# ZhonghuaYi/FocusFlow_official

Measured on AMD Instinct MI355X. Metric: frame-pairs/sec FF-RAFT 384x512 iters=12, higher is better.
Workload: dtype f32 via fp16x3 split operands on the f16 MFMA pipe (f32 accumulate, fp32-level accuracy); 1 GPU; FF-RAFT forward (test_mode), 8 pairs/GPU 384x512, iters=12, fp32 correlation pyramid, random-init weights, ORB-like masks (BASELINE configs[1]); pairs_per_gpu=8, corr_pyramid=fp32, conv_precision=f16x3, hipgraph=False, skip_unused_upsample=False, parallelism=dp1 (independent shards, no collective)

## Files before the change

### focusflow_official_amd/csrc/conv_patch.hip

```cpp
#include <algorithm>
#include <cstdlib>
#include "ff_common.h"

namespace {

typedef float f32x16 __attribute__((ext_vector_type(16)));
typedef float f32x4 __attribute__((ext_vector_type(4)));
typedef _Float16 f16x8 __attribute__((ext_vector_type(8)));
typedef _Float16 f16x4 __attribute__((ext_vector_type(4)));

constexpr int TW = 16, ROWB = 128;
constexpr int ROWP = 144;
__device__ __forceinline__ int PI16(int i) { return (i >= 4 && i < 12) ? 2 * (i - 4) : (i < 4 ? 2 * i + 1 : 2 * (i - 12) + 9); }
__device__ __forceinline__ int KG16(int g) { return ((g & 1) << 1) | (g >> 1); }


struct PArgs {
    FFConvParams p;
    int Cin, nci;
    int tiles_x, tiles_y, n_tiles;
    long long w_row_bytes;
    int nci_split;
};

__device__ __forceinline__ void split4(const f32x4 v, f16x4& h0, f16x4& h1) {
#pragma unroll
    for (int j = 0; j < 4; ++j) {
        const _Float16 a = (_Float16)v[j];
        h0[j] = a;
        h1[j] = (_Float16)(v[j] - (float)a);
    }
}

template <int TERMS, int NITEM, int TM, int TN, int ABL, int WB, bool PIN = false, bool INORM = false, bool SPLITK = false, bool MF16 = false, int EPI = 0, bool STATS = false>
__device__ __forceinline__ void conv_patch_body(const PArgs& a) {
    constexpr int TH = 4 * TM, BN = 64 * TN, NW = 2 * TN;
    extern __shared__ __attribute__((aligned(16))) char smem[];
    const FFConvParams& p = a.p;
    float xs, xinv;
    ff::input_scale(p.x_amax, xs, xinv);
    xs *= ff::XSPLIT; xinv *= ff::SPLIT_INV;
    const int KH = p.KH, KW = p.KW, PH = TH + KH - 1, PW = TW + KW - 1, NPIX = PH * PW;
    char* sP = smem;
    char* sW = smem + ((NPIX * ROWP + 255) & ~255);

    const int tid = threadIdx.x, lane = tid & 63, wave = tid >> 6;
    const int wm = wave >> 1, wn = wave & 1;
    const int H = p.H, W = p.W;
    int bid = blockIdx.x;
    const int nt = bid % a.n_tiles; bid /= a.n_tiles;
    const int tx = bid % a.tiles_x; bid /= a.tiles_x;
    const int ty = bid % a.tiles_y;
    const int bimg = bid / a.tiles_y;
    const int y0 = ty * TH, x0 = tx * TW, n0 = nt * BN;

    const long long pix_total = (long long)p.B * H * W;
    __amdgpu_buffer_rsrc_t rs0 = __builtin_amdgcn_make_buffer_rsrc(const_cast<float*>(p.x[0]), 0, (int)(pix_total * p.x_ld[0] * 4), 0x00020000);
    __amdgpu_buffer_rsrc_t rs1 = __builtin_amdgcn_make_buffer_rsrc(const_cast<float*>(p.x[1] ? p.x[1] : p.x[0]), 0, p.x[1] ? (int)(pix_total * p.x_ld[1] * 4) : 0, 0x00020000);
    __amdgpu_buffer_rsrc_t rs2 = __builtin_amdgcn_make_buffer_rsrc(const_cast<float*>(p.x[2] ? p.x[2] : p.x[0]), 0, p.x[2] ? (int)(pix_total * p.x_ld[2] * 4) : 0, 0x00020000);
    __amdgpu_buffer_rsrc_t rsw = __builtin_amdgcn_make_buffer_rsrc(const_cast<float*>(p.w), 0, (int)((long long)p.Cout * a.w_row_bytes), 0x00020000);
    const int c0 = p.x_c[0], c01 = p.x_c[0] + p.x_c[1];

    int ppix[NITEM];
    int prow[NITEM];
#pragma unroll
    for (int i = 0; i < NITEM; ++i) {
        const int item = tid + 256 * i;
        const int px = item >> 3;
        ppix[i] = -1;
        prow[i] = px;
        if (px < NPIX) {
            const int yy = y0 - p.pad_h + px / PW, xx = x0 - p.pad_w + px % PW;
            if ((unsigned)yy < (unsigned)H && (unsigned)xx < (unsigned)W) ppix[i] = (bimg * H + yy) * W + xx;
        }
    }
    const int kq = tid & 7;
    int woff[NW];
#pragma unroll
    for (int i = 0; i < NW; ++i) {
        const int n = n0 + (tid >> 3) + 32 * i;
        woff[i] = n < p.Cout ? (int)(n * a.w_row_bytes) + kq * 16 : 0x7fffffff;
    }

    f32x4 rp[NITEM], rw[NW];
    f32x4 nmul = {1.f, 1.f, 1.f, 1.f}, nadd = {0.f, 0.f, 0.f, 0.f};
    auto load_patch = [&](int c) {
        int ci0 = c * 32;
        if (INORM) {
            const long long t = (long long)bimg * a.Cin + ci0 + kq * 4;
            nmul = *reinterpret_cast<const f32x4*>(p.in_scale + t);
            nadd = *reinterpret_cast<const f32x4*>(p.in_shift + t);
        }
        __amdgpu_buffer_rsrc_t rs;
        int ldb;
        if (ci0 < c0) { rs = rs0; ldb = p.x_ld[0] * 4; }
        else if (ci0 < c01) { rs = rs1; ldb = p.x_ld[1] * 4; ci0 -= c0; }
        else { rs = rs2; ldb = p.x_ld[2] * 4; ci0 -= c01; }
        const int cib = (ci0 + kq * 4) * 4;
#pragma unroll
        for (int i = 0; i < NITEM; ++i) {
            const int off = ppix[i] >= 0 ? ppix[i] * ldb + cib : 0x7fffffff;
            rp[i] = __builtin_bit_cast(f32x4, __builtin_amdgcn_raw_buffer_load_b128(rs, off, 0, 0));
        }
    };
    auto store_patch = [&]() {
        const int pc = MF16 ? KG16(kq >> 1) : kq >> 1, half = (kq & 1) * 8;
#pragma unroll
        for (int i = 0; i < NITEM; ++i) {
            const int row = prow[i];
            if (row < NPIX) {
                f16x4 h0, h1;
                f32x4 v = rp[i];
                if (INORM) {
                    v = __builtin_elementwise_fma(v, nmul, nadd);
                    if (p.in_act == FF_ACT_RELU) {
#pragma unroll
                        for (int j = 0; j < 4; ++j) v[j] = v[j] < 0.f ? 0.f : v[j];
                    }
                    if (ppix[i] < 0) v = (f32x4){0.f, 0.f, 0.f, 0.f};
                }
                split4(v * xs, h0, h1);
                *reinterpret_cast<f16x4*>(sP + row * ROWP + pc * 16 + half) = h0;
                if (TERMS == 3) *reinterpret_cast<f16x4*>(sP + row * ROWP + 64 + pc * 16 + half) = h1;
            }
        }
    };
    auto load_w = [&](int kc) {
#pragma unroll
        for (int i = 0; i < NW; ++i)
            rw[i] = __builtin_bit_cast(f32x4, __builtin_amdgcn_raw_buffer_load_b128(rsw, woff[i], kc * ROWB, 0));
    };
    auto store_w = [&](int buf) {
        char* d = sW + buf * BN * ROWP;
#pragma unroll
        for (int i = 0; i < NW; ++i) {
            const int row = (tid >> 3) + 32 * i;
            if (MF16) *reinterpret_cast<f32x4*>(d + ((row & ~15) + PI16(row & 15)) * ROWP + ((kq & 4) | KG16(kq & 3)) * 16) = rw[i];
            else *reinterpret_cast<f32x4*>(d + row * ROWP + kq * 16) = rw[i];
        }
    };

    if constexpr (MF16) {
        constexpr int NU = 2 * TM, NV = 2 * TN;
        f32x4 acc[NV][NU];
#pragma unroll
        for (int v = 0; v < NV; ++v)
#pragma unroll
            for (int u = 0; u < NU; ++u) acc[v][u] = (f32x4){0.f, 0.f, 0.f, 0.f};
        const int i16 = lane & 15, g16 = lane >> 4, pcol = PI16(i16);
        const int ntaps = KH * KW;
        const char* xbase = sP + ((wm * NU) * PW + pcol) * ROWP + KG16(g16) * 16;
        const int wrow0 = (wn * TN * 32 + PI16(i16)) * ROWP + KG16(g16) * 16;
        const int c_beg = SPLITK ? (int)blockIdx.y * a.nci_split : 0;
        const int c_end = SPLITK ? min(c_beg + a.nci_split, a.nci) : a.nci;
        load_patch(c_beg);
        load_w(c_beg);
        int wbuf = 0;
        for (int c = c_beg; c < c_end; ++c) {
            __syncthreads();
            store_patch();
            store_w(wbuf);
            __syncthreads();
            if (c + 1 < c_end) load_patch(c + 1);
            for (int tap = 0; tap < ntaps; ++tap) {
                const bool last = tap + 1 == ntaps;
                const int next_kc = last ? (c + 1) : (tap + 1) * a.nci + c;
                if (!(last && c + 1 == c_end)) load_w(last ? c + 1 : next_kc);
                if (PIN) __builtin_amdgcn_sched_barrier(0);
                const int dy = tap / KW, dx = tap - dy * KW;
                const char* pa = xbase + (dy * PW + dx) * ROWP;
                const char* cW = sW + wbuf * BN * ROWP + wrow0;
                f16x8 w0[NV], w1[NV];
#pragma unroll
                for (int v = 0; v < NV; ++v) {
                    w0[v] = *reinterpret_cast<const f16x8*>(cW + v * 16 * ROWP);
                    if (TERMS == 3) w1[v] = *reinterpret_cast<const f16x8*>(cW + v * 16 * ROWP + 64);
                }
#pragma unroll
                for (int u = 0; u < NU; ++u) {
                    const f16x8 xa = *reinterpret_cast<const f16x8*>(pa + u * PW * ROWP);
                    f16x8 xb;
                    if (TERMS == 3) xb = *reinterpret_cast<const f16x8*>(pa + u * PW * ROWP + 64);
#pragma unroll
                    for (int v = 0; v < NV; ++v) {
                        acc[v][u] = __builtin_amdgcn_mfma_f32_16x16x32_f16(w0[v], xa, acc[v][u], 0, 0, 0);
                        if (TERMS == 3) {
                            acc[v][u] = __builtin_amdgcn_mfma_f32_16x16x32_f16(w1[v], xa, acc[v][u], 0, 0, 0);
                            acc[v][u] = __builtin_amdgcn_mfma_f32_16x16x32_f16(w0[v], xb, acc[v][u], 0, 0, 0);
                        }
                    }
                }
                if (!last) {
                    if (WB == 1) __syncthreads();
                    store_w(WB == 1 ? 0 : wbuf ^ 1);
                    __syncthreads();
                    if (WB == 2) wbuf ^= 1;
                }
            }
            if (WB == 2) wbuf ^= 1;
        }
        const int x = x0 + pcol;
        const bool vec_y = (p.y_ld & 3) == 0 && ff::aligned16(p.y);
        const bool vec_r = !p.res || ((p.res_ld & 3) == 0 && ff::aligned16(p.res));
#pragma unroll
        for (int v = 0; v < NV; ++v) {
            const int n4 = n0 + wn * TN * 32 + v * 16 + g16 * 4;
            if (n4 >= p.Cout) continue;
            const bool full = n4 + 3 < p.Cout;
            if constexpr (SPLITK) {
                float* ws = p.splitk_ws + (long long)blockIdx.y * pix_total * p.Cout;
#pragma unroll
                for (int u = 0; u < NU; ++u) {
                    const int y = y0 + wm * NU + u;
                    if (y >= H || x >= W) continue;
                    float* d = ws + (((long long)bimg * H + y) * W + x) * p.Cout + n4;
                    if (full && (p.Cout & 3) == 0) *reinterpret_cast<f32x4*>(d) = acc[v][u] * xinv;
                    else {
#pragma unroll
                        for (int r = 0; r < 4; ++r)
                            if (n4 + r < p.Cout) d[r] = acc[v][u][r] * xinv;
                    }
                }
                continue;
            }
            f32x4 bias = {0.f, 0.f, 0.f, 0.f}, cs = {1.f, 1.f, 1.f, 1.f}, ct = {0.f, 0.f, 0.f, 0.f};
#pragma unroll
            for (int r = 0; r < 4; ++r) {
                const int n = min(n4 + r, p.Cout - 1);
                if (p.bias) bias[r] = p.bias[n];
                if (p.ch_scale) { cs[r] = p.ch_scale[n]; ct[r] = p.ch_shift[n]; }
            }
            f32x4 vv[NU], rr[NU];
            long long po[NU];
#pragma unroll
            for (int u = 0; u < NU; ++u) {
                const int y = y0 + wm * NU + u;
                po[u] = (y < H && x < W) ? ((long long)bimg * H + y) * W + x : -1;
                f32x4 t = acc[v][u] * xinv + bias;
                t *= p.out_scale;
                if (p.ch_scale) t = t * cs + ct;
#pragma unroll
                for (int r = 0; r < 4; ++r) t[r] = ff::apply_act(t[r], p.act);
                vv[u] = t;
            }
            if (p.res) {
#pragma unroll
                for (int u = 0; u < NU; ++u) {
                    rr[u] = (f32x4){0.f, 0.f, 0.f, 0.f};
                    if (po[u] < 0) continue;
                    const float* rp2 = p.res + po[u] * p.res_ld + n4;
                    if (full && vec_r) rr[u] = *reinterpret_cast<const f32x4*>(rp2);
                    else {
#pragma unroll
                        for (int r = 0; r < 4; ++r)
                            if (n4 + r < p.Cout) rr[u][r] = rp2[r];
                    }
                }
#pragma unroll
                for (int u = 0; u < NU; ++u)
#pragma unroll
                    for (int r = 0; r < 4; ++r) vv[u][r] = ff::apply_act(vv[u][r] + rr[u][r], p.act_res);
            }
            if constexpr (EPI == FF_EP_GRU_RH) {
                if (n4 >= p.ep_split) {
#pragma unroll
                    for (int u = 0; u < NU; ++u) rr[u] = po[u] >= 0 ? *reinterpret_cast<const f32x4*>(p.ep_a + po[u] * p.ep_a_ld + (n4 - p.ep_split)) : (f32x4){0.f, 0.f, 0.f, 0.f};
#pragma unroll
                    for (int u = 0; u < NU; ++u)
#pragma unroll
                        for (int r = 0; r < 4; ++r) vv[u][r] = __fmul_rn(vv[u][r], rr[u][r]);
                }
            }
            if constexpr (EPI == FF_EP_GRU_BLEND) {
                f32x4 zz[NU];
#pragma unroll
                for (int u = 0; u < NU; ++u) {
                    zz[u] = po[u] >= 0 ? *reinterpret_cast<const f32x4*>(p.ep_a + po[u] * p.ep_a_ld + n4) : (f32x4){0.f, 0.f, 0.f, 0.f};
                    rr[u] = po[u] >= 0 ? *reinterpret_cast<const f32x4*>(p.ep_b + po[u] * p.ep_b_ld + n4) : (f32x4){0.f, 0.f, 0.f, 0.f};
                }
#pragma unroll
                for (int u = 0; u < NU; ++u)
#pragma unroll
                    for (int r = 0; r < 4; ++r)
                        vv[u][r] = __fadd_rn(__fmul_rn(__fsub_rn(1.f, zz[u][r]), rr[u][r]), __fmul_rn(zz[u][r], vv[u][r]));
            }
#pragma unroll
            for (int u = 0; u < NU; ++u) {
                if (po[u] < 0) continue;
                float* d = p.y + po[u] * p.y_ld + n4;
                if (full && vec_y) *reinterpret_cast<f32x4*>(d) = vv[u];
                else {
#pragma unroll
                    for (int r = 0; r < 4; ++r)
                        if (n4 + r < p.Cout) d[r] = vv[u][r];
                }
            }
        }
        return;
    }

    f32x16 acc[TM][TN];
#pragma unroll
    for (int i = 0; i < TM; ++i)
#pragma unroll
        for (int j = 0; j < TN; ++j)
#pragma unroll
            for (int r = 0; r < 16; ++r) acc[i][j][r] = 0.f;

    const int li = lane & 31, lh = lane >> 5;
    const int rot = (KW - 1) & 15;
    const int lrow = li >> 4, lcol = ((li & 15) - lrow * rot) & 15;
    const int ntaps = KH * KW;
    const int brow = wn * TN * 32 + li;
    const char* abase[TM];
#pragma unroll
    for (int t = 0; t < TM; ++t) abase[t] = sP + (((wm * TM + t) * 2 + lrow) * PW + lcol) * ROWP + lh * 16;

    f16x8 abl_f;
#pragma unroll
    for (int i = 0; i < 8; ++i) abl_f[i] = (_Float16)(0.37f + 0.01f * (float)((lane * 7 + i * 3) & 31));
    const int c_beg = SPLITK ? (int)blockIdx.y * a.nci_split : 0;
    const int c_end = SPLITK ? min(c_beg + a.nci_split, a.nci) : a.nci;
    load_patch(c_beg);
    load_w(c_beg);
    int wbuf = 0;
    for (int c = c_beg; c < c_end; ++c) {
        __syncthreads();
        if (ABL != 6 || c == c_beg) store_patch();
        store_w(wbuf);
        __syncthreads();
        if (c + 1 < c_end && ABL != 6) load_patch(c + 1);
        for (int tap = 0; tap < ntaps; ++tap) {
            const bool last = tap + 1 == ntaps;
            const int next_kc = last ? (c + 1) : (tap + 1) * a.nci + c;
            if (!(last && c + 1 == c_end) && ABL != 1 && ABL != 2) load_w(last ? c + 1 : next_kc);
            if (PIN) __builtin_amdgcn_sched_barrier(0);
            const int dy = tap / KW, dx = tap - dy * KW;
            const int tapoff = (dy * PW + dx) * ROWP;
            const char* cW = sW + wbuf * BN * ROWP + brow * ROWP + lh * 16;
#pragma unroll
            for (int s = 0; s < 2; ++s) {
                f16x8 a0[TM], a1[TM], b0[TN], b1[TN];
                if constexpr (ABL == 5) {
#pragma unroll
                    for (int t = 0; t < TM; ++t) { a0[t] = abl_f; a1[t] = abl_f; }
#pragma unroll
                    for (int j = 0; j < TN; ++j) { b0[j] = abl_f; b1[j] = abl_f; }
                    asm volatile("" : "+v"(abl_f));
                } else {
#pragma unroll
                for (int t = 0; t < TM; ++t) {
                    const char* pa = abase[t] + tapoff;
                    a0[t] = *reinterpret_cast<const f16x8*>(pa + s * 32);
                    if (TERMS == 3) a1[t] = *reinterpret_cast<const f16x8*>(pa + 64 + s * 32);
                }
#pragma unroll
                for (int j = 0; j < TN; ++j) {
                    b0[j] = *reinterpret_cast<const f16x8*>(cW + j * 32 * ROWP + s * 32);
                    if (TERMS == 3) b1[j] = *reinterpret_cast<const f16x8*>(cW + j * 32 * ROWP + 64 + s * 32);
                }
                }
#pragma unroll
                for (int t = 0; t < TM; ++t)
#pragma unroll
                    for (int j = 0; j < TN; ++j) {
                        if constexpr (ABL == 3) {
                            asm volatile("" :: "v"(a0[t]), "v"(b0[j]));
                            if (TERMS == 3) asm volatile("" :: "v"(a1[t]), "v"(b1[j]));
                            continue;
                        }
                        acc[t][j] = __builtin_amdgcn_mfma_f32_32x32x16_f16(a0[t], b0[j], acc[t][j], 0, 0, 0);
                        if (TERMS == 3) {
                            acc[t][j] = __builtin_amdgcn_mfma_f32_32x32x16_f16(a0[t], b1[j], acc[t][j], 0, 0, 0);
                            acc[t][j] = __builtin_amdgcn_mfma_f32_32x32x16_f16(a1[t], b0[j], acc[t][j], 0, 0, 0);
                        }
                    }
            }
            if (!last && ABL != 2) {
                if (WB == 1 && ABL != 4) __syncthreads();
                store_w(WB == 1 ? 0 : wbuf ^ 1);
                if (ABL != 4) __syncthreads();
                if (WB == 2) wbuf ^= 1;
            }
        }
        if (WB == 2) wbuf ^= 1;
    }

    if constexpr (SPLITK) {
        float* ws = p.splitk_ws + (long long)blockIdx.y * pix_total * p.Cout;
#pragma unroll
        for (int j = 0; j < TN; ++j) {
            const int n = n0 + (wn * TN + j) * 32 + li;
            if (n >= p.Cout) continue;
#pragma unroll
            for (int t = 0; t < TM; ++t)
#pragma unroll
                for (int r = 0; r < 16; ++r) {
                    const int pi = (r & 3) + 8 * (r >> 2) + 4 * lh;
                    const int y = y0 + (wm * TM + t) * 2 + (pi >> 4), x = x0 + ((pi - (pi >> 4) * rot) & 15);
                    if (y < H && x < W) ws[(((long long)bimg * H + y) * W + x) * p.Cout + n] = acc[t][j][r] * xinv;
                }
        }
        return;
    }
#pragma unroll
    for (int j = 0; j < TN; ++j) {
        const int n = n0 + (wn * TN + j) * 32 + li;
        if (n >= p.Cout) continue;
        const float bias = p.bias ? p.bias[n] : 0.f;
        const float cs = p.ch_scale ? p.ch_scale[n] : 1.f;
        const float ct = p.ch_scale ? p.ch_shift[n] : 0.f;
        const bool split_out = p.y_fmt == FF_FMT_SPLIT && n >= p.y_fmt_from;
        float st_p = 0.f, st_s1 = 0.f, st_s2 = 0.f, st_n = 0.f;
#pragma unroll
        for (int t = 0; t < TM; ++t) {
            float vv[16];
#pragma unroll
            for (int r = 0; r < 16; ++r) {
                float v = acc[t][j][r] * xinv + bias;
                v *= p.out_scale;
                if (p.ch_scale) v = v * cs + ct;
                vv[r] = ff::apply_act(v, p.act);
            }
            if (p.res) {
                float rr[16];
#pragma unroll
                for (int r = 0; r < 16; ++r) {
                    const int pi = (r & 3) + 8 * (r >> 2) + 4 * lh;
                    const int y = y0 + (wm * TM + t) * 2 + (pi >> 4), x = x0 + ((pi - (pi >> 4) * rot) & 15);
                    rr[r] = (y < H && x < W) ? p.res[(((long long)bimg * H + y) * W + x) * p.res_ld + n] : 0.f;
                }
#pragma unroll
                for (int r = 0; r < 16; ++r) vv[r] = ff::apply_act(vv[r] + rr[r], p.act_res);
            }
#pragma unroll
            for (int r = 0; r < 16; ++r) {
                const int pi = (r & 3) + 8 * (r >> 2) + 4 * lh;
                const int y = y0 + (wm * TM + t) * 2 + (pi >> 4), x = x0 + ((pi - (pi >> 4) * rot) & 15);
                if (y >= H || x >= W) continue;
                const long long pix = ((long long)bimg * H + y) * W + x;
                if (split_out) ff::store_split1(p.y + pix * p.y_ld, n, vv[r]);
                else p.y[pix * p.y_ld + n] = vv[r];
            }
            if constexpr (STATS) {
                if (y0 + TH <= H && x0 + TW <= W) {
                    if (t == 0) st_p = vv[0];
#pragma unroll
                    for (int r = 0; r < 16; ++r) {
                        const float d = vv[r] - st_p;
                        st_s1 += d;
                        st_s2 = fmaf(d, d, st_s2);
                    }
                    st_n += 16.f;
                } else {
#pragma unroll
                    for (int r = 0; r < 16; ++r) {
                        const int pi = (r & 3) + 8 * (r >> 2) + 4 * lh;
                        const int y = y0 + (wm * TM + t) * 2 + (pi >> 4), x = x0 + ((pi - (pi >> 4) * rot) & 15);
                        if (y >= H || x >= W) continue;
                        if (st_n == 0.f) st_p = vv[r];
                        const float d = vv[r] - st_p;
                        st_s1 += d;
                        st_s2 = fmaf(d, d, st_s2);
                        st_n += 1.f;
                    }
                }
            }
        }
        if constexpr (STATS) {
            const float p2 = __shfl_xor(st_p, 32), s2 = __shfl_xor(st_s1, 32), q2 = __shfl_xor(st_s2, 32), n2 = __shfl_xor(st_n, 32);
            if (lh == 0) {
                const float pv = st_n > 0.f ? st_p : p2, d = p2 - pv;
                const float s1 = st_s1 + s2 + n2 * d;
                const float q1 = st_s2 + q2 + 2.f * d * s2 + n2 * d * d;
                const int part = (ty * a.tiles_x + tx) * 2 + wm;
                const int nparts = a.tiles_y * a.tiles_x * 2;
                *reinterpret_cast<f32x4*>(p.stats_part + (((long long)bimg * nparts + part) * p.Cout + n) * 4) = (f32x4){pv, s1, q1, st_n + n2};
            }
        }
    }
}

template <int TERMS, int NITEM, int TM, int TN, int ABL = 0, int WB = 2>
__global__ __launch_bounds__(256) void conv_patch_kernel(const PArgs a) { conv_patch_body<TERMS, NITEM, TM, TN, ABL, WB>(a); }
template <int TERMS, int NITEM, int TM, int TN, int OCC, bool PIN = true, int ABL = 0, bool INORM = false, bool SPLITK = false, bool MF16 = false, int EPI = 0, bool STATS = false>
__global__ __launch_bounds__(256) __attribute__((amdgpu_waves_per_eu(OCC, OCC))) void conv_patch_kernel_occ(const PArgs a) { conv_patch_body<TERMS, NITEM, TM, TN, ABL, 1, PIN, INORM, SPLITK, MF16, EPI, STATS>(a); }

__global__ __launch_bounds__(256) void splitk_finish_kernel(const FFConvParams p, int splits, long long npix) {
    const long long total = npix * p.Cout;
    for (long long i = blockIdx.x * 256ll + threadIdx.x; i < total; i += (long long)gridDim.x * 256) {
        const long long m = i / p.Cout;
        const int n = (int)(i - m * p.Cout);
        float v = 0.f;
        for (int s = 0; s < splits; ++s) v += p.splitk_ws[(long long)s * total + i];
        v += p.bias ? p.bias[n] : 0.f;
        v *= p.out_scale;
        if (p.ch_scale) v = v * p.ch_scale[n] + p.ch_shift[n];
        v = ff::apply_act(v, p.act);
        if (p.res) v = ff::apply_act(v + p.res[m * p.res_ld + n], p.act_res);
        p.y[m * p.y_ld + n] = v;
    }
}

template <int TERMS, int NITEM, int TM, int TN, int OCC>
int launch_occ(const PArgs& a, size_t lds, hipStream_t s) {
    const long long blocks = (long long)a.p.B * a.tiles_y * a.tiles_x * a.n_tiles;
    static const bool mf16 = ff::tune_env("FF_MFMA16") && atoi(ff::tune_env("FF_MFMA16")) == 1;
    if (a.p.stats_part) {
        if (a.p.in_scale) conv_patch_kernel_occ<TERMS, NITEM, TM, TN, OCC, true, 0, true, false, false, 0, true><<<(unsigned)blocks, 256, lds, s>>>(a);
        else conv_patch_kernel_occ<TERMS, NITEM, TM, TN, OCC, true, 0, false, false, false, 0, true><<<(unsigned)blocks, 256, lds, s>>>(a);
        return ff::check_launch("ff_conv2d_fwd(patch, statistics)");
    }
    if (a.p.ep_mode) {
        if (a.p.ep_mode == FF_EP_GRU_RH) conv_patch_kernel_occ<TERMS, NITEM, TM, TN, OCC, true, 0, false, false, true, FF_EP_GRU_RH><<<(unsigned)blocks, 256, lds, s>>>(a);
        else conv_patch_kernel_occ<TERMS, NITEM, TM, TN, OCC, true, 0, false, false, true, FF_EP_GRU_BLEND><<<(unsigned)blocks, 256, lds, s>>>(a);
        return ff::check_launch("ff_conv2d_fwd(patch, GRU epilogue)");
    }
    if (mf16) {
        if (a.p.splitk > 1) {
            const int splits = (a.nci + a.nci_split - 1) / a.nci_split;
            conv_patch_kernel_occ<TERMS, NITEM, TM, TN, OCC, true, 0, false, true, true><<<dim3((unsigned)blocks, splits), 256, lds, s>>>(a);
            const long long npix = (long long)a.p.B * a.p.H * a.p.W, total = npix * a.p.Cout;
            splitk_finish_kernel<<<(unsigned)std::min<long long>((total + 255) / 256, 2048), 256, 0, s>>>(a.p, splits, npix);
            return ff::check_launch("ff_conv2d_fwd(patch, split-K)");
        }
        if (a.p.in_scale) conv_patch_kernel_occ<TERMS, NITEM, TM, TN, OCC, true, 0, true, false, true><<<(unsigned)blocks, 256, lds, s>>>(a);
        else conv_patch_kernel_occ<TERMS, NITEM, TM, TN, OCC, true, 0, false, false, true><<<(unsigned)blocks, 256, lds, s>>>(a);
        return ff::check_launch("ff_conv2d_fwd(patch)");
    }
    if (a.p.splitk > 1) {
        const int splits = (a.nci + a.nci_split - 1) / a.nci_split;
        conv_patch_kernel_occ<TERMS, NITEM, TM, TN, OCC, true, 0, false, true><<<dim3((unsigned)blocks, splits), 256, lds, s>>>(a);
        const long long npix = (long long)a.p.B * a.p.H * a.p.W, total = npix * a.p.Cout;
        splitk_finish_kernel<<<(unsigned)std::min<long long>((total + 255) / 256, 2048), 256, 0, s>>>(a.p, splits, npix);
        return ff::check_launch("ff_conv2d_fwd(patch, split-K)");
    }
    static const bool pin = !(ff::tune_env("FF_PATCH_PIN") && atoi(ff::tune_env("FF_PATCH_PIN")) == 0);
    if (a.p.in_scale) {
        conv_patch_kernel_occ<TERMS, NITEM, TM, TN, OCC, true, 0, true><<<(unsigned)blocks, 256, lds, s>>>(a);
        return ff::check_launch("ff_conv2d_fwd(patch)");
    }
#ifdef FF_LAB
    static const int oabl = getenv("FF_PATCH_ABLATE") ? atoi(getenv("FF_PATCH_ABLATE")) : 0;
#define FF_OCC_ABL(ENV_, ABL_) \
    if (oabl == ENV_) { conv_patch_kernel_occ<TERMS, NITEM, TM, TN, OCC, true, ABL_><<<(unsigned)blocks, 256, lds, s>>>(a); return ff::check_launch("ff_conv2d_fwd(patch)"); }
    FF_OCC_ABL(4, 4) FF_OCC_ABL(11, 1) FF_OCC_ABL(12, 2) FF_OCC_ABL(13, 3) FF_OCC_ABL(15, 5) FF_OCC_ABL(16, 6)
#undef FF_OCC_ABL
#endif
    if (!pin) {
        conv_patch_kernel_occ<TERMS, NITEM, TM, TN, OCC, false><<<(unsigned)blocks, 256, lds, s>>>(a);
        return ff::check_launch("ff_conv2d_fwd(patch)");
    }
    conv_patch_kernel_occ<TERMS, NITEM, TM, TN, OCC><<<(unsigned)blocks, 256, lds, s>>>(a);
    return ff::check_launch("ff_conv2d_fwd(patch)");
}

template <int NITEM, int TM, int TN, int OCC>
int launch_occ_f16(const PArgs& a, size_t lds, hipStream_t s) {
    const long long blocks = (long long)a.p.B * a.tiles_y * a.tiles_x * a.n_tiles;
    if (a.p.stats_part) {
        if (a.p.in_scale) conv_patch_kernel_occ<1, NITEM, TM, TN, OCC, true, 0, true, false, false, 0, true><<<(unsigned)blocks, 256, lds, s>>>(a);
        else conv_patch_kernel_occ<1, NITEM, TM, TN, OCC, true, 0, false, false, false, 0, true><<<(unsigned)blocks, 256, lds, s>>>(a);
        return ff::check_launch("ff_conv2d_fwd(patch, f16, statistics)");
    }
    if (a.p.ep_mode) {
        if (a.p.ep_mode == FF_EP_GRU_RH) conv_patch_kernel_occ<1, NITEM, TM, TN, OCC, true, 0, false, false, true, FF_EP_GRU_RH><<<(unsigned)blocks, 256, lds, s>>>(a);
        else conv_patch_kernel_occ<1, NITEM, TM, TN, OCC, true, 0, false, false, true, FF_EP_GRU_BLEND><<<(unsigned)blocks, 256, lds, s>>>(a);
        return ff::check_launch("ff_conv2d_fwd(patch, f16, GRU epilogue)");
    }
    if (a.p.splitk > 1) {
        const int splits = (a.nci + a.nci_split - 1) / a.nci_split;
        conv_patch_kernel_occ<1, NITEM, TM, TN, OCC, true, 0, false, true><<<dim3((unsigned)blocks, splits), 256, lds, s>>>(a);
        const long long npix = (long long)a.p.B * a.p.H * a.p.W, total = npix * a.p.Cout;
        splitk_finish_kernel<<<(unsigned)std::min<long long>((total + 255) / 256, 2048), 256, 0, s>>>(a.p, splits, npix);
        return ff::check_launch("ff_conv2d_fwd(patch, f16, split-K)");
    }
    if (a.p.in_scale) conv_patch_kernel_occ<1, NITEM, TM, TN, OCC, true, 0, true><<<(unsigned)blocks, 256, lds, s>>>(a);
    else conv_patch_kernel_occ<1, NITEM, TM, TN, OCC><<<(unsigned)blocks, 256, lds, s>>>(a);
    return ff::check_launch("ff_conv2d_fwd(patch, f16)");
}

template <int TERMS, int NITEM, int TM, int TN, int ABL = 0, int WB = 2>
int launch(const PArgs& a, size_t lds, hipStream_t s) {
    static bool once = false;
    if (!once) {
        (void)hipFuncSetAttribute(reinterpret_cast<const void*>(&conv_patch_kernel<TERMS, NITEM, TM, TN, ABL, WB>), hipFuncAttributeMaxDynamicSharedMemorySize, 96 * 1024);
        once = true;
    }
    const long long blocks = (long long)a.p.B * a.tiles_y * a.tiles_x * a.n_tiles;
    conv_patch_kernel<TERMS, NITEM, TM, TN, ABL, WB><<<(unsigned)blocks, 256, lds, s>>>(a);
    return ff::check_launch("ff_conv2d_fwd(patch)");
}

}

namespace ff {
int conv2d_fwd_patch(const FFConvParams& p, int cin, hipStream_t s) {
    static const bool enabled = !ff::tune_env("FF_NO_PATCH_CONV");
    static const bool dbg = ff::tune_env("FF_DEBUG_DISPATCH") != nullptr;
    if (dbg) fprintf(stderr, "[ff] patch? en=%d stride=%d dil=%d,%d groups=%d k=%dx%d pad=%d,%d cin=%d xc=%d,%d,%d fmt=%d\n", (int)enabled, p.stride,
                     p.dil_h, p.dil_w, p.groups, p.KH, p.KW, p.pad_h, p.pad_w, cin, p.x_c[0], p.x_c[1], p.x_c[2], p.w_format);
    if (!enabled) return 1;
    const int dlh = p.dil_h ? p.dil_h : 1, dlw = p.dil_w ? p.dil_w : 1;
    if (p.stride != 1 || dlh != 1 || dlw != 1 || p.groups != 1) return 1;
    if (p.KH % 2 == 0 || p.KW % 2 == 0 || p.pad_h != p.KH / 2 || p.pad_w != p.KW / 2 || p.KH > 7 || p.KW > 7) return 1;
    if (p.KH * p.KW < 3) return 1;
    if (cin % 32) return 1;
    long long max_bytes = 0;
    for (int i = 0; i < FF_MAX_SEG; ++i) {
        if (p.x_c[i] % 32) return 1;
        if (p.x_c[i]) max_bytes = std::max(max_bytes, (long long)p.B * p.H * p.W * p.x_ld[i] * 4);
    }
    PArgs a;
    a.p = p;
    a.Cin = cin;
    a.nci = cin / 32;
    a.tiles_x = (p.W + TW - 1) / TW;
    a.w_row_bytes = (long long)((p.KH * p.KW * cin + 31) / 32) * ROWB;
    max_bytes = std::max(max_bytes, (long long)p.Cout * a.w_row_bytes);
    if (max_bytes >= (1ll << 31)) return 1;
    static const int force_th = ff::tune_env("FF_PATCH_TH") ? atoi(ff::tune_env("FF_PATCH_TH")) : 0;
    static const int force_tn = ff::tune_env("FF_PATCH_TN") ? atoi(ff::tune_env("FF_PATCH_TN")) : 0;
    auto nblocks = [&](int th, int tn) { return (long long)p.B * ((p.H + th - 1) / th) * a.tiles_x * ((p.Cout + 64 * tn - 1) / (64 * tn)); };
    int th = nblocks(8, 1) < 512 ? 4 : 8, tn = 1;
    if (force_th) th = force_th;
    if (force_tn) tn = force_tn;
    a.tiles_y = (p.H + th - 1) / th;
    a.n_tiles = (p.Cout + 64 * tn - 1) / (64 * tn);
    const int npix = (th + p.KH - 1) * (TW + p.KW - 1);
    static const int lds_pad = ff::tune_env("FF_PATCH_LDS_PAD") ? atoi(ff::tune_env("FF_PATCH_LDS_PAD")) : 0;
    const int nitem = (npix * 8 + 255) / 256;
    const bool t3 = p.w_format == FF_W_F16X3;
    static const int wb1 = ff::tune_env("FF_PATCH_WB1") ? atoi(ff::tune_env("FF_PATCH_WB1")) : 3;
    const bool occ = (t3 || p.w_format == FF_W_F16) && tn == 1 && ((th == 8 && nitem <= 6 && (wb1 & 1)) || (th == 4 && nitem <= 4 && (wb1 & 2)));
    const size_t lds = ((npix * ROWP + 255) & ~255) + (occ ? 1 : 2) * 64 * tn * ROWP + lds_pad;
    if (lds > 96 * 1024) return 1;
#ifdef FF_LAB
    static const int abl = getenv("FF_PATCH_ABLATE") ? atoi(getenv("FF_PATCH_ABLATE")) : 0;
    if (abl >= 1 && abl <= 3 && th == 8 && tn == 1 && nitem <= 6 && t3) {
        if (abl == 1) return launch<3, 6, 2, 1, 1>(a, lds, s);
        if (abl == 2) return launch<3, 6, 2, 1, 2>(a, lds, s);
        return launch<3, 6, 2, 1, 3>(a, lds, s);
    }
#endif
    if (p.y_fmt != FF_FMT_F32) {
        static const bool mf16 = ff::tune_env("FF_MFMA16") && atoi(ff::tune_env("FF_MFMA16")) == 1;
        if (!occ || p.ep_mode || p.splitk > 1 || mf16) return 1;
    }
    if (!(occ && th == 4 && p.splitk > 1 && p.splitk_ws && !p.in_scale && !p.res2)) a.p.splitk = 0;
    a.nci_split = a.p.splitk > 1 ? (a.nci + a.p.splitk - 1) / a.p.splitk : a.nci;
    if (p.stats_part && (!occ || a.p.splitk > 1 || p.ep_mode))
        return ff::fail(FF_EINVAL, "ff_conv2d_fwd: stats_part: ask ff_conv2d_stats_parts first (this convolution cannot produce statistics)");
    if (p.ep_mode) {
        if (!occ || a.p.splitk > 1 || p.in_scale || p.Cout % 4) return ff::fail(FF_EINVAL, "ff_conv2d_fwd: ep_mode needs the f16x3 patch kernel's 8x16 / 4x16 tiles (got %dx%d kernel, Cin %d, Cout %d)", p.KH, p.KW, cin, p.Cout);
    }
    if (occ && !t3) return th == 8 ? launch_occ_f16<6, 2, 1, 4>(a, lds, s) : launch_occ_f16<4, 1, 1, 5>(a, lds, s);
    if (occ) return th == 8 ? launch_occ<3, 6, 2, 1, 4>(a, lds, s) : launch_occ<3, 4, 1, 1, 5>(a, lds, s);
    if (p.in_scale) return 1;
#define FF_PATCH_CASE(TH_, TN_, NI_) \
    if (th == TH_ && tn == TN_ && nitem <= NI_) return t3 ? launch<3, NI_, TH_ / 4, TN_>(a, lds, s) : launch<1, NI_, TH_ / 4, TN_>(a, lds, s);
    FF_PATCH_CASE(8, 1, 6) FF_PATCH_CASE(8, 1, 10)
    FF_PATCH_CASE(4, 1, 4) FF_PATCH_CASE(4, 1, 8)
    FF_PATCH_CASE(8, 2, 6) FF_PATCH_CASE(8, 2, 10)
    FF_PATCH_CASE(4, 2, 4) FF_PATCH_CASE(4, 2, 8)
    FF_PATCH_CASE(16, 1, 11) FF_PATCH_CASE(16, 1, 16)
#undef FF_PATCH_CASE
    return 1;
}

int conv2d_stats_parts(const FFConvParams& p, int cin) {
    static const bool enabled = !ff::tune_env("FF_NO_PATCH_CONV") && !(getenv("FF_CONV_STATS") && atoi(getenv("FF_CONV_STATS")) == 0);
    if (!enabled || (p.w_format != FF_W_F16X3 && p.w_format != FF_W_F16) || p.res2 || p.ep_mode || p.x_amax) return 0;
    const int dlh = p.dil_h ? p.dil_h : 1, dlw = p.dil_w ? p.dil_w : 1;
    if (p.stride != 1 || dlh != 1 || dlw != 1 || p.groups != 1) return 0;
    if (p.KH % 2 == 0 || p.KW % 2 == 0 || p.pad_h != p.KH / 2 || p.pad_w != p.KW / 2 || p.KH > 7 || p.KW > 7 || p.KH * p.KW < 3) return 0;
    if (cin % 32) return 0;
    for (int i = 0; i < FF_MAX_SEG; ++i)
        if (p.x_c[i] % 32) return 0;
    if (ff::tune_env("FF_PATCH_TH") || ff::tune_env("FF_PATCH_TN") || ff::tune_env("FF_PATCH_WB1")) return 0;
    long long max_bytes = (long long)p.Cout * ((p.KH * p.KW * cin + 31) / 32) * ROWB;
    for (int i = 0; i < FF_MAX_SEG; ++i)
        if (p.x_c[i]) max_bytes = std::max(max_bytes, (long long)p.B * p.H * p.W * p.x_ld[i] * 4);
    if (max_bytes >= (1ll << 31)) return 0;
    const int tiles_x = (p.W + TW - 1) / TW, n_tiles = (p.Cout + 63) / 64;
    const int th = (long long)p.B * ((p.H + 7) / 8) * tiles_x * n_tiles < 512 ? 4 : 8;
    const int npix = (th + p.KH - 1) * (TW + p.KW - 1), nitem = (npix * 8 + 255) / 256;
    if (!((th == 8 && nitem <= 6) || (th == 4 && nitem <= 4))) return 0;
    if (th == 4 && p.splitk > 1 && p.splitk_ws) return 0;
    return ((p.H + th - 1) / th) * tiles_x * 2;
}

int conv2d_splitk_hint(const FFConvParams& p, int cin) {
    static const bool enabled = !ff::tune_env("FF_NO_PATCH_CONV") && !(ff::tune_env("FF_SPLITK") && atoi(ff::tune_env("FF_SPLITK")) == 0);
    if (!enabled || p.w_format != FF_W_F16X3 || p.in_scale || p.res2) return 0;
    const int dlh = p.dil_h ? p.dil_h : 1, dlw = p.dil_w ? p.dil_w : 1;
    if (p.stride != 1 || dlh != 1 || dlw != 1 || p.groups != 1) return 0;
    if (p.KH % 2 == 0 || p.KW % 2 == 0 || p.pad_h != p.KH / 2 || p.pad_w != p.KW / 2 || p.KH * p.KW < 3) return 0;
    if (cin % 32) return 0;
    for (int i = 0; i < FF_MAX_SEG; ++i)
        if (p.x_c[i] % 32) return 0;
    const int tiles_x = (p.W + TW - 1) / TW, n_tiles = (p.Cout + 63) / 64;
    if ((long long)p.B * ((p.H + 7) / 8) * tiles_x * n_tiles >= 512) return 0;
    const int npix = (4 + p.KH - 1) * (TW + p.KW - 1);
    if ((npix * 8 + 255) / 256 > 4) return 0;
    const long long blocks = (long long)p.B * ((p.H + 3) / 4) * tiles_x * n_tiles;
    const int nci = cin / 32;
    if (blocks > 256 || nci < 6 || nci * p.KH * p.KW <= (p.splitk < 0 ? 36 : 72)) return 0;
    const int splits = (int)std::min<long long>(std::min(16, nci / 2), 768 / blocks);
    return splits >= 2 ? splits : 0;
}
}
```

Before: 623.5 frame-pairs/s.

## Stage conv epilogue through LDS for vectorized 16-byte NHWC stores

Adds a vectorized epilogue path in the patch convolution kernel. Each wave transposes its MFMA accumulator tile through a per-wave LDS staging buffer, so every lane then owns four consecutive channels and can issue 16-byte loads of the residual and 16-byte stores of the output instead of scattered 4-byte accesses. The activation is specialized at compile time through a switch over integral constants. This adds LDS traffic, wave barriers and code size, and it only applies when alignment and stride conditions hold.

```diff
diff --git a/focusflow_official_amd/csrc/conv_patch.hip b/focusflow_official_amd/csrc/conv_patch.hip
--- a/focusflow_official_amd/csrc/conv_patch.hip
+++ b/focusflow_official_amd/csrc/conv_patch.hip
@@ -1,5 +1,6 @@
 #include <algorithm>
 #include <cstdlib>
+#include <type_traits>
 #include "ff_common.h"
 
 namespace {
@@ -29,6 +30,27 @@
         const _Float16 a = (_Float16)v[j];
         h0[j] = a;
         h1[j] = (_Float16)(v[j] - (float)a);
+    }
+}
+
+template <class F>
+__device__ __forceinline__ void act_switch(int act, F&& f) {
+    switch (act) {
+        case FF_ACT_RELU: f(std::integral_constant<int, FF_ACT_RELU>{}); break;
+        case FF_ACT_SIGMOID: f(std::integral_constant<int, FF_ACT_SIGMOID>{}); break;
+        case FF_ACT_TANH: f(std::integral_constant<int, FF_ACT_TANH>{}); break;
+        case FF_ACT_LEAKY: f(std::integral_constant<int, FF_ACT_LEAKY>{}); break;
+        default: f(std::integral_constant<int, FF_ACT_NONE>{});
+    }
+}
+template <int ACT, bool CS>
+__device__ __forceinline__ void tile_values(const f32x16& acc, float xinv, float bias, float out_scale, float cs, float ct, float (&vv)[16]) {
+#pragma unroll
+    for (int r = 0; r < 16; ++r) {
+        float v = acc[r] * xinv + bias;
+        v *= out_scale;
+        if (CS) v = v * cs + ct;
+        vv[r] = ff::apply_act(v, ACT);
     }
 }
 
@@ -400,6 +422,85 @@
                     const int y = y0 + (wm * TM + t) * 2 + (pi >> 4), x = x0 + ((pi - (pi >> 4) * rot) & 15);
                     if (y < H && x < W) ws[(((long long)bimg * H + y) * W + x) * p.Cout + n] = acc[t][j][r] * xinv;
                 }
+        }
+        return;
+    }
+    const bool vec = !STATS && (p.y_ld & 3) == 0 && ff::aligned16(p.y) && (p.Cout & 3) == 0 && (!p.res || ((p.res_ld & 3) == 0 && ff::aligned16(p.res))) &&
+                     (p.y_fmt != FF_FMT_SPLIT || (p.y_fmt_from & 3) == 0) &&
+                     (long long)(TH + 1) * W * max(p.y_ld, p.res_ld) * 4 < (1ll << 31);
+    if (vec) {
+        __syncthreads();
+        const int uw = __builtin_amdgcn_readfirstlane(wave), uwm = uw >> 1, uwn = uw & 1;
+        char* stg = smem + uw * 4096;
+        char* stg_w = stg + lh * 512 + li * 4;
+        const char* stg_r = stg + lane * 16;
+        const int q = lane >> 3, c4 = (lane & 7) * 4;
+        const int col[4] = {q, q + 8, (q - rot) & 15, (q + 8 - rot) & 15};
+        unsigned yo[4], ro[4];
+#pragma unroll
+        for (int k = 0; k < 4; ++k) {
+            const unsigned px = (unsigned)((k >> 1) * W + col[k]);
+            yo[k] = (px * (unsigned)p.y_ld + (unsigned)c4) * 4u;
+            ro[k] = (px * (unsigned)p.res_ld + (unsigned)c4) * 4u;
+        }
+        const int ty0 = y0 + uwm * TM * 2;
+        const long long pix0 = ((long long)bimg * H + ty0) * W + x0;
+        const bool interior = y0 + TH <= H && x0 + TW <= W;
+#pragma unroll
+        for (int j = 0; j < TN; ++j) {
+            const int nb = n0 + (uwn * TN + j) * 32;
+            if (nb >= p.Cout) continue;
+            const int n = nb + li, nc = min(n, p.Cout - 1);
+            const float bias = p.bias ? p.bias[nc] : 0.f;
+            const float cs = p.ch_scale ? p.ch_scale[nc] : 1.f;
+            const float ct = p.ch_scale ? p.ch_shift[nc] : 0.f;
+            char* yb = reinterpret_cast<char*>(p.y + pix0 * p.y_ld + nb);
+            const char* rb = p.res ? reinterpret_cast<const char*>(p.res + pix0 * p.res_ld + nb) : nullptr;
+            const bool sp = p.y_fmt == FF_FMT_SPLIT && nb + c4 >= p.y_fmt_from;
+            const bool whole = interior && nb + 32 <= p.Cout;
+#pragma unroll
+            for (int t = 0; t < TM; ++t) {
+                float vv[16];
+                act_switch(p.act, [&](auto A) {
+                    if (p.ch_scale) tile_values<decltype(A)::value, true>(acc[t][j], xinv, bias, p.out_scale, cs, ct, vv);
+                    else tile_values<decltype(A)::value, false>(acc[t][j], xinv, bias, p.out_scale, cs, ct, vv);
+                });
+#pragma unroll
+                for (int r = 0; r < 16; ++r) *reinterpret_cast<float*>(stg_w + ((r & 3) + 8 * (r >> 2)) * 128) = vv[r];
+                __builtin_amdgcn_fence(__ATOMIC_RELEASE, "wavefront");
+                __builtin_amdgcn_wave_barrier();
+                __builtin_amdgcn_fence(__ATOMIC_ACQUIRE, "wavefront");
+                f32x4 pc[4];
+#pragma unroll
+                for (int k = 0; k < 4; ++k) pc[k] = *reinterpret_cast<const f32x4*>(stg_r + k * 1024);
+                __builtin_amdgcn_fence(__ATOMIC_RELEASE, "wavefront");
+                __builtin_amdgcn_wave_barrier();
+                __builtin_amdgcn_fence(__ATOMIC_ACQUIRE, "wavefront");
+                bool ok[4];
+#pragma unroll
+                for (int k = 0; k < 4; ++k)
+                    ok[k] = whole || (ty0 + t * 2 + (k >> 1) < H && x0 + col[k] < W && nb + c4 < p.Cout);
+                const unsigned tby = (unsigned)(t * 2 * W) * (unsigned)p.y_ld * 4u, tbr = (unsigned)(t * 2 * W) * (unsigned)p.res_ld * 4u;
+                if (p.res) {
+                    f32x4 rr[4];
+#pragma unroll
+                    for (int k = 0; k < 4; ++k)
+                        rr[k] = ok[k] ? *reinterpret_cast<const f32x4*>(rb + (size_t)(ro[k] + tbr)) : (f32x4){0.f, 0.f, 0.f, 0.f};
+                    act_switch(p.act_res, [&](auto A) {
+#pragma unroll
+                        for (int k = 0; k < 4; ++k)
+#pragma unroll
+                            for (int e = 0; e < 4; ++e) pc[k][e] = ff::apply_act(pc[k][e] + rr[k][e], decltype(A)::value);
+                    });
+                }
+#pragma unroll
+                for (int k = 0; k < 4; ++k) {
+                    if (!ok[k]) continue;
+                    if (sp) {
+                        ff::store_split4(reinterpret_cast<float*>(yb + (size_t)(yo[k] + tby - (unsigned)c4 * 4u)) - nb, nb + c4, pc[k]);
+                    } else *reinterpret_cast<f32x4*>(yb + (size_t)(yo[k] + tby)) = pc[k];
+                }
+            }
         }
         return;
     }
```

New measurement: 628.4 frame-pairs/s, median of 6. Within noise of the previous version (+0.8%).
